# sp-uhh/audio-visual-vad

Hardware: AMD Instinct MI355X
Metric: AV frame-pairs/sec (fwd+bwd) (higher is better)
Workload: dtype f32; 1 GPU; AV_net fused training step (WaveNet-W0 encoder + ResNet-18 trunk + concat + 2xLSTM1024 + FC, masked BCE, backward, RCCL all-reduce, fused Adam): BASELINE configs[3]/[4] per-GPU shard; per_gpu_frame_pairs=1024, global_frame_pairs=1024, sequences_per_gpu=64, parallelism=dp1, reserved_cus=0, reported_block=median

## Files before the change

audio-visual-vad_amd/csrc/common.h:

```cpp
#pragma once
#include <hip/hip_runtime.h>
#include <stdint.h>
#include <atomic>

#include "avvad.h"

typedef float f32x16 __attribute__((ext_vector_type(16)));
typedef float f32x4 __attribute__((ext_vector_type(4)));

#include <stdio.h>
#define AVVAD_LAUNCH_CHECK()                                                                      \
  do {                                                                                            \
    hipError_t e_ = hipGetLastError();                                                            \
    if (e_ != hipSuccess) {                                                                       \
      fprintf(stderr, "avvad: HIP error '%s' after launch at %s:%d\n", hipGetErrorString(e_), __FILE__, __LINE__); \
      return AVVAD_ELAUNCH;                                                                       \
    }                                                                                             \
  } while (0)

#define AVVAD_ENTER() (void)hipGetLastError()

struct AvvadTune {
  int igemm_variant;
  int no_streamk;
  int kmajor;
  int lstm_no_fused_step;
  int lstm_no_persistent;
  int no_stem_kernel;
  int no_tall;
  int wn_no_fused_tail;
  int wn_no_tail_pair;
  int wn_no_fused_wgrad;
  int no_fixup1;
  int no_buf;
  int wn_flat;
  int wn_dx;
  int wn_grid;
  int wn_bwd_t;
  int bf16;
  int stagger;
  int cls_cap;
  int no_cls;
  int no_fused_stats;
  int no_s2_cls;
  int no_conv64;
  int bwd_max_cus;
  int max_cus;
};
AvvadTune& avvad_tune();
struct BwdCuCap {
  int saved;
  BwdCuCap() : saved(avvad_tune().max_cus) {
    const int b = avvad_tune().bwd_max_cus;
    if (b > 0 && (saved <= 0 || b < saved)) avvad_tune().max_cus = b;
  }
  ~BwdCuCap() { avvad_tune().max_cus = saved; }
};
static inline int grid_cus() {
  const int m = avvad_tune().max_cus;
  return (m > 0 && m < 256) ? m : 256;
}

template <auto Kernel>
int allow_large_lds(size_t bytes, size_t limit) {
  if (bytes <= 64 * 1024) return AVVAD_OK;
// ... 78 lines not shown
```

audio-visual-vad_amd/csrc/misc.hip:

```cpp
#include "common.h"

extern "C" const char* avvad_version(void) { return "avvad-hip 0.1 (gfx950, fp32 MFMA)"; }
extern "C" int avvad_abi_version(void) { return AVVAD_ABI_VERSION; }

#include <stdlib.h>
#include <string.h>
namespace {
struct OptName { const char* name; const char* env; int AvvadTune::*field; };
const OptName kOpts[] = {
    {"igemm_variant", "AVVAD_IGEMM_VARIANT", &AvvadTune::igemm_variant},
    {"no_streamk", "AVVAD_NO_STREAMK", &AvvadTune::no_streamk},
    {"kmajor", "AVVAD_KMAJOR", &AvvadTune::kmajor},
    {"lstm_no_fused_step", "AVVAD_LSTM_NO_FUSED_STEP", &AvvadTune::lstm_no_fused_step},
    {"lstm_no_persistent", "AVVAD_LSTM_NO_PERSISTENT", &AvvadTune::lstm_no_persistent},
    {"no_stem_kernel", "AVVAD_NO_STEM_KERNEL", &AvvadTune::no_stem_kernel},
    {"no_tall", "AVVAD_NO_TALL", &AvvadTune::no_tall},
    {"wn_no_fused_tail", "AVVAD_WN_NO_FUSED_TAIL", &AvvadTune::wn_no_fused_tail},
    {"wn_no_tail_pair", "AVVAD_WN_NO_TAIL_PAIR", &AvvadTune::wn_no_tail_pair},
    {"wn_no_fused_wgrad", "AVVAD_WN_NO_FUSED_WGRAD", &AvvadTune::wn_no_fused_wgrad},
    {"wn_bwd_t", "AVVAD_WN_BWD_T", &AvvadTune::wn_bwd_t},
    {"no_buf", "AVVAD_NO_BUF", &AvvadTune::no_buf},
    {"no_fixup1", "AVVAD_NO_FIXUP1", &AvvadTune::no_fixup1},
    {"no_conv64", "AVVAD_NO_CONV64", &AvvadTune::no_conv64},
    {"no_s2_cls", "AVVAD_NO_S2_CLS", &AvvadTune::no_s2_cls},
    {"wn_flat", "AVVAD_WN_FLAT", &AvvadTune::wn_flat},
    {"wn_grid", "AVVAD_WN_GRID", &AvvadTune::wn_grid},
    {"wn_dx", "AVVAD_WN_DX", &AvvadTune::wn_dx},
    {"bf16", "AVVAD_BF16", &AvvadTune::bf16},
    {"no_fused_stats", "AVVAD_NO_FUSED_STATS", &AvvadTune::no_fused_stats},
    {"no_cls", "AVVAD_NO_CLS", &AvvadTune::no_cls},
    {"cls_cap", "AVVAD_CLS_CAP", &AvvadTune::cls_cap},
    {"stagger", "AVVAD_STAGGER", &AvvadTune::stagger},
    {"max_cus", "AVVAD_MAX_CUS", &AvvadTune::max_cus},
    {"bwd_max_cus", "AVVAD_BWD_MAX_CUS", &AvvadTune::bwd_max_cus},
};
int parse_opt(const char* name, const char* v) {
  if (!strcmp(name, "igemm_variant")) return v[0] == 'd' ? 0 : (v[0] == 's' ? 1 : (v[0] == 'w' ? 2 : atoi(v)));
  if (!strcmp(name, "no_streamk")) return v[0] == 'a' ? 1 : (v[0] >= '0' && v[0] <= '9' && !v[1] ? 10 + (v[0] - '0') : atoi(v));
  if (!strcmp(name, "max_cus") || !strcmp(name, "bwd_max_cus") || !strcmp(name, "wn_flat") || !strcmp(name, "wn_grid") || !strcmp(name, "wn_dx") || !strcmp(name, "wn_bwd_t") || !strcmp(name, "no_fixup1") || !strcmp(name, "cls_cap")) return atoi(v);
  return (v[0] && strcmp(v, "0")) ? 1 : 0;
}
}

AvvadTune& avvad_tune() {
  static AvvadTune t = [] {
    AvvadTune x;
    memset(&x, 0, sizeof(x));
    x.igemm_variant = -1;
    for (const OptName& o : kOpts) {
      const char* v = getenv(o.env);
      if (v && v[0]) x.*(o.field) = parse_opt(o.name, v);
    }
// ... 281 lines not shown
```

audio-visual-vad_amd/csrc/wavenet.hip:

```cpp
#include "gemm_api.h"
#include "wn_block.h"
#include "wn_tail.h"

namespace {

static inline int grid1(long n) { long b = (n + 255) / 256; return (int)(b > 8192 ? 8192 : (b < 1 ? 1 : b)); }

__global__ void conv1d_fwd_generic(const float* __restrict__ x, const float* __restrict__ w, const float* __restrict__ bias,
                                   const float* __restrict__ res, float* __restrict__ y, int B, int Cin, int Cout, int Lin,
                                   int Lout, int fw, int dil, int relu_in, int res_off, int res_L) {
  const long n = (long)B * Cout * Lout;
  for (long i = (long)blockIdx.x * blockDim.x + threadIdx.x; i < n; i += (long)gridDim.x * blockDim.x) {
    const int t = (int)(i % Lout);
    const int co = (int)((i / Lout) % Cout);
    const int b = (int)(i / ((long)Lout * Cout));
    float acc = bias ? bias[co] : 0.f;
    const float* xb = x + (long)b * Cin * Lin + t;
    const float* wr = w + (long)co * Cin * fw;
    for (int ci = 0; ci < Cin; ++ci)
      for (int k = 0; k < fw; ++k) {
        float v = xb[(long)ci * Lin + k * dil];
        if (relu_in) v = fmaxf(v, 0.f);
        acc = fmaf(wr[ci * fw + k], v, acc);
      }
// ... 449 lines not shown
    const float* sp = s_in + (long)b * 32 * Lin + (ok ? t : 0);
    const float* rp = dS_out + (long)b * 32 * Lo + (okr ? t - dil : 0);
#pragma unroll
    for (int r = 0; r < 16; ++r) { svn[r] = sp[(long)mfma32_row(r, lh) * Lin]; rvn[r] = rp[(long)mfma32_row(r, lh) * Lo]; }
  };
  const TileWalk tw = xcd_walk(ntiles);
  if (tw.first < tw.last) issue(tw.first);
  for (long tile = tw.first; tile < tw.last; tile += tw.stride) {
    const TilePos p = tile_pos(tile, tiles_per_seq, li, Lin);
    const int b = p.b, t = p.t;
    const bool ok = p.ok;
    const int to = t - lh * dil;
    const bool okz = ok && to >= 0 && to < Lo;
    const bool okr = ok && t >= dil;
    float dz[32], sv[16], rv[16];
#pragma unroll
    for (int s = 0; s < 32; ++s) dz[s] = okz ? dzn[s] : 0.f;
#pragma unroll
    for (int r = 0; r < 16; ++r) { sv[r] = svn[r]; rv[r] = okr ? rvn[r] : 0.f; }
    issue(tile + tw.stride);
    f32x16 acc;
#pragma unroll
    for (int r = 0; r < 16; ++r) acc[r] = 0.f;
#pragma unroll
    for (int s = 0; s < 32; ++s) acc = mfma32(wt[s], dz[s], acc);
    float* op = dS_in + (long)b * 32 * Lin + t;
#pragma unroll
    for (int r = 0; r < 16; ++r)
      if (ok) op[(long)mfma32_row(r, lh) * Lin] = (sv[r] > 0.f ? acc[r] : 0.f) + rv[r];
  }
}

struct DxTile { float dz[32], sv[16], rv[16]; };
template <bool RESIDENT>
__device__ __forceinline__ void wn_block_bwd_dx_body(float* wl, const float* __restrict__ DZ, const float* __restrict__ s_in,
                                                     const float* __restrict__ dS_out, const float* __restrict__ w_dil,
                                                     float* __restrict__ dS_in, int B, int Lin, int dil) {
  const int lane = threadIdx.x & 63;
  const int li = lane & 31, lh = lane >> 5;
  const int Lo = Lin - dil;
  const int tiles_per_seq = tiles_per_sequence<32>(Lin);
  const int ntiles = B * tiles_per_seq;
  const float* wtl = wl + li * 2 + lh;
  const int rowL = Lin * 4, rowO = Lo * 4;
  float wt[32];
  auto issue = [&](int tile, DxTile& n) __attribute__((always_inline)) {
    const TilePos p = tile_pos(RESIDENT && tile >= ntiles ? ntiles - 1 : tile, tiles_per_seq, li, Lin);
    const int t = p.t;
    const int to = t - lh * dil;
    const bool okz = p.ok && to >= 0 && to < Lo;
    const bool okr = p.ok && t >= dil;
    const __amdgpu_buffer_rsrc_t rz = brsrc(DZ + (long)p.b * 32 * Lo, 32 * rowO);
    const __amdgpu_buffer_rsrc_t rs = brsrc(s_in + (long)p.b * 32 * Lin, 32 * rowL);
    const __amdgpu_buffer_rsrc_t rg = brsrc(dS_out + (long)p.b * 32 * Lo, 32 * rowO);
    const int offz = okz ? to * 4 : BUF_OOB;
    const int offs = p.ok ? t * 4 + 4 * lh * rowL : BUF_OOB;
    const int offg = okr ? (t - dil) * 4 + 4 * lh * rowO : BUF_OOB;
#pragma unroll
    for (int s = 0; s < 32; ++s) n.dz[s] = bload(rz, offz, s * rowO);
#pragma unroll
    for (int r = 0; r < 16; ++r) { n.sv[r] = bload(rs, offs, mfma32_row(r, 0) * rowL); n.rv[r] = bload(rg, offg, mfma32_row(r, 0) * rowO); }
  };
  auto compute = [&](int tile, const DxTile& c) __attribute__((always_inline)) {
    const TilePos p = tile_pos(tile, tiles_per_seq, li, Lin);
    const __amdgpu_buffer_rsrc_t ro = brsrc(dS_in + (long)p.b * 32 * Lin, 32 * rowL);
    const int offs = p.ok ? p.t * 4 + 4 * lh * rowL : BUF_OOB;
    f32x16 acc;
#pragma unroll
    for (int r = 0; r < 16; ++r) acc[r] = 0.f;
#pragma unroll
    for (int s = 0; s < 32; ++s) acc = mfma32(RESIDENT ? wt[s] : wtl[WIMG_DIL_PITCH * s], c.dz[s], acc);
#pragma unroll
    for (int r = 0; r < 16; ++r) bstore((c.sv[r] > 0.f ? acc[r] : 0.f) + c.rv[r], ro, offs, mfma32_row(r, 0) * rowL);
  };
  const TileWalkI w = xcd_walk_i(ntiles);
  DxTile ta, tb;
  if (RESIDENT && w.first < w.last) issue(w.first, ta);
  stage_w_dil(wl, w_dil, threadIdx.x, 256);
  __syncthreads();
  if (RESIDENT) {
#pragma unroll
    for (int s = 0; s < 32; ++s) wt[s] = wtl[WIMG_DIL_PITCH * s];
    pingpong_tiles<false>(w, ta, tb, issue, compute);
  } else {
    plain_tiles<false, DxTile>(w, issue, compute);
  }
}

__global__ void __launch_bounds__(256)
    wn_block_bwd_dx_buf(const float* __restrict__ DZ, const float* __restrict__ s_in, const float* __restrict__ dS_out,
                        const float* __restrict__ w_dil, float* __restrict__ dS_in, int B, int Lin, int dil) {
  __shared__ float wl[WIMG_DIL_SIZE];
  wn_block_bwd_dx_body<true>(wl, DZ, s_in, dS_out, w_dil, dS_in, B, Lin, dil);
}

__global__ void __launch_bounds__(256, 4)
    wn_block_bwd_dx_occ(const float* __restrict__ DZ, const float* __restrict__ s_in, const float* __restrict__ dS_out,
                        const float* __restrict__ w_dil, float* __restrict__ dS_in, int B, int Lin, int dil) {
  __shared__ float wl[WIMG_DIL_SIZE];
  wn_block_bwd_dx_body<false>(wl, DZ, s_in, dS_out, w_dil, dS_in, B, Lin, dil);
}

constexpr int WG_SLAB = 3 * 1024 + 64;
constexpr int WG_MAXBLK = 512;

__global__ void __launch_bounds__(256)
    wn_block_wgrad_mfma(const float* __restrict__ dS, const float* __restrict__ Z, const float* __restrict__ DZ,
                        const float* __restrict__ s_in, float* __restrict__ slab, int B, int Lin, int dil) {
// ... 47 lines not shown
    xpose(v0, ok, false, fa);
#pragma unroll
    for (int q = 0; q < 16; ++q) bs_dz += fa[q];
    xpose(v1, ok, true, fb);
#pragma unroll
    for (int q = 0; q < 16; ++q) acc0 = mfma32(fa[q], fb[q], acc0);
    xpose(v2, ok, true, fb);
#pragma unroll
    for (int q = 0; q < 16; ++q) acc1 = mfma32(fa[q], fb[q], acc1);
    xpose(v3, ok, false, fa);
#pragma unroll
    for (int q = 0; q < 16; ++q) bs_ds += fa[q];
    xpose(v4, ok, true, fb);
#pragma unroll
    for (int q = 0; q < 16; ++q) acc2 = mfma32(fa[q], fb[q], acc2);
  }

  __syncthreads();
#pragma unroll
  for (int r = 0; r < 16; ++r) {
    const int row = mfma32_row(r, lh);
    atomicAdd(&red[row * 32 + li], acc0[r]);
    atomicAdd(&red[1024 + row * 32 + li], acc1[r]);
    atomicAdd(&red[2048 + row * 32 + li], acc2[r]);
  }
  atomicAdd(&red[3072 + li], bs_dz);
  atomicAdd(&red[3104 + li], bs_ds);
  __syncthreads();
  float* out = slab + (long)blockIdx.x * WG_SLAB;
  for (int i = threadIdx.x; i < WG_SLAB; i += 256) out[i] = red[i];
}

struct DzwTile { float g[16], x[32]; };
template <bool RESIDENT>
__device__ __forceinline__ void wn_block_bwd_dz_wgrad_body(float* tiles, float* red, float* wl, float* wtl,
                                                           const float* __restrict__ dS, const float* __restrict__ w_dil,
                                                           const float* __restrict__ b_dil, const float* __restrict__ w_dense,
                                                           const float* __restrict__ s_in, float* __restrict__ DZ,
                                                           float* __restrict__ slab, int B, int Lin, int dil) {
  const int lane = threadIdx.x & 63, wave = threadIdx.x >> 6;
  const int li = lane & 31, lh = lane >> 5;
  const int Lo = Lin - dil;
  const int tiles_per_seq = tiles_per_sequence<32>(Lo);
  const int ntiles = B * tiles_per_seq;
  float* T = tiles + wave * 2 * 1056;
  float* T1 = T + 1056;
  float* Th = T + lh * 1056;
  stage_w_dil(wl, w_dil, threadIdx.x, 256);
  stage_bias(wl + WIMG_DIL_SIZE, b_dil, threadIdx.x);
  if (RESIDENT) stage_w_dense(T, w_dense, lane, 64);
  else stage_w_dense(wtl, w_dense, threadIdx.x, 256);
  for (int i = threadIdx.x; i < WG_SLAB; i += 256) red[i] = 0.f;
  __syncthreads();
  const float* wtp = (RESIDENT ? T : wtl) + lh * WIMG_DENSE_PITCH + li;
  const float* wdp = wl + li * WIMG_DIL_PITCH + lh;
  const float* bzl = wl + WIMG_DIL_SIZE + 4 * lh;
  float wt[16], wd[32];
  if (RESIDENT) {
#pragma unroll
    for (int s = 0; s < 16; ++s) wt[s] = wtp[2 * WIMG_DENSE_PITCH * s];
#pragma unroll
    for (int s = 0; s < 32; ++s) wd[s] = wdp[2 * s];
  }
  __builtin_amdgcn_wave_barrier();

  f32x16 acc0, acc1, acc2;
#pragma unroll
  for (int r = 0; r < 16; ++r) { acc0[r] = 0.f; acc1[r] = 0.f; acc2[r] = 0.f; }
  float bs_dz = 0.f, bs_ds = 0.f;
  const int rowL = Lin * 4, rowO = Lo * 4;

  auto issue = [&](int tile, DzwTile& n) __attribute__((always_inline)) {
    const TilePos p = tile_pos(tile < ntiles ? tile : ntiles - 1, tiles_per_seq, li, Lo);
    const __amdgpu_buffer_rsrc_t rg = brsrc(dS + (long)p.b * 32 * Lo, 32 * rowO);
    const __amdgpu_buffer_rsrc_t rx = brsrc(s_in + (long)p.b * 32 * Lin, 32 * rowL);
    const int offg = p.ok ? p.t * 4 + lh * rowO : BUF_OOB;
    const int offx = p.ok ? (p.t + lh * dil) * 4 : BUF_OOB;
#pragma unroll
    for (int q = 0; q < 16; ++q) n.g[q] = bload(rg, offg, 2 * q * rowO);
#pragma unroll
    for (int c = 0; c < 32; ++c) n.x[c] = bload(rx, offx, c * rowL);
  };
  auto compute = [&](int tidx, const DzwTile& c) __attribute__((always_inline)) {
    const TilePos p = tile_pos(tidx, tiles_per_seq, li, Lo);
    const int offo = p.ok ? p.t * 4 + 4 * lh * rowO : BUF_OOB;
    const __amdgpu_buffer_rsrc_t rz = brsrc(DZ + (long)p.b * 32 * Lo, 32 * rowO);
    float x[32];
#pragma unroll
    for (int s = 0; s < 32; ++s) x[s] = relu1(c.x[s]);
    f32x16 z;
#pragma unroll
    for (int r = 0; r < 16; ++r) z[r] = bzl[mfma32_row(r, 0)];
#pragma unroll
    for (int s = 0; s < 32; ++s) z = mfma32(RESIDENT ? wd[s] : wdp[2 * s], x[s], z);
    f32x16 acc;
#pragma unroll
    for (int r = 0; r < 16; ++r) acc[r] = 0.f;
#pragma unroll
    for (int q = 0; q < 16; ++q) acc = mfma32(RESIDENT ? wt[q] : wtp[2 * WIMG_DENSE_PITCH * q], c.g[q], acc);
    float f0[16], f1[16];
    __builtin_amdgcn_wave_barrier();
#pragma unroll
    for (int r = 0; r < 16; ++r) {
      const float dz = z[r] > 0.f ? acc[r] : 0.f;
      bstore(dz, rz, offo, mfma32_row(r, 0) * rowO);
      T[mfma32_row(r, lh) * 33 + li] = dz;
    }
    __builtin_amdgcn_wave_barrier();
#pragma unroll
    for (int q = 0; q < 16; ++q) { f0[q] = T[li * 33 + 2 * q + lh]; bs_dz += f0[q]; }
    __builtin_amdgcn_wave_barrier();
#pragma unroll
    for (int s = 0; s < 32; ++s) Th[s * 33 + li] = x[s];
    __builtin_amdgcn_wave_barrier();
#pragma unroll
    for (int q = 0; q < 16; ++q) f1[q] = T[li * 33 + 2 * q + lh];
#pragma unroll
    for (int q = 0; q < 16; ++q) acc0 = mfma32(f0[q], f1[q], acc0);
#pragma unroll
    for (int q = 0; q < 16; ++q) f1[q] = T1[li * 33 + 2 * q + lh];
#pragma unroll
    for (int q = 0; q < 16; ++q) acc1 = mfma32(f0[q], f1[q], acc1);
    __builtin_amdgcn_wave_barrier();
#pragma unroll
    for (int q = 0; q < 16; ++q) T[(2 * q + lh) * 33 + li] = c.g[q];
#pragma unroll
    for (int r = 0; r < 16; ++r) T1[mfma32_row(r, lh) * 33 + li] = relu1(z[r]);
    __builtin_amdgcn_wave_barrier();
#pragma unroll
    for (int q = 0; q < 16; ++q) { f0[q] = T[li * 33 + 2 * q + lh]; bs_ds += f0[q]; }
#pragma unroll
    for (int q = 0; q < 16; ++q) f1[q] = T1[li * 33 + 2 * q + lh];
#pragma unroll
    for (int q = 0; q < 16; ++q) acc2 = mfma32(f0[q], f1[q], acc2);
    __builtin_amdgcn_wave_barrier();
  };
  const TileWalkI w = xcd_walk_i(ntiles);
  DzwTile ta, tb;
  if (RESIDENT) {
    if (w.first < w.last) issue(w.first, ta);
    pingpong_tiles<true>(w, ta, tb, issue, compute);
  } else {
    plain_tiles<true, DzwTile>(w, issue, compute);
  }

  for (int wv = 0; wv < 4; ++wv) {
    __syncthreads();
    if (wave == wv) {
#pragma unroll
      for (int r = 0; r < 16; ++r) {
        const int row = mfma32_row(r, lh);
        red[row * 32 + li] += acc0[r];
        red[1024 + row * 32 + li] += acc1[r];
        red[2048 + row * 32 + li] += acc2[r];
      }
      if (lh == 0) { red[3072 + li] += bs_dz; red[3104 + li] += bs_ds; }
      __builtin_amdgcn_wave_barrier();
      if (lh == 1) { red[3072 + li] += bs_dz; red[3104 + li] += bs_ds; }
    }
  }
  __syncthreads();
  float* out = slab + (long)blockIdx.x * WG_SLAB;
  for (int i = threadIdx.x; i < WG_SLAB; i += 256) out[i] = red[i];
}

__global__ void __launch_bounds__(256)
    wn_block_bwd_dz_wgrad_mfma(const float* __restrict__ dS, const float* __restrict__ w_dil, const float* __restrict__ b_dil,
                               const float* __restrict__ w_dense, const float* __restrict__ s_in, float* __restrict__ DZ,
                               float* __restrict__ slab, int B, int Lin, int dil) {
  __shared__ float tile[4 * 2 * 32 * 33];
  __shared__ float red[WG_SLAB];
  __shared__ float wl[WIMG_DIL_SIZE + 32];
  wn_block_bwd_dz_wgrad_body<true>(tile, red, wl, nullptr, dS, w_dil, b_dil, w_dense, s_in, DZ, slab, B, Lin, dil);
}

__global__ void __launch_bounds__(256, 2)
    wn_block_bwd_dz_wgrad_occ(const float* __restrict__ dS, const float* __restrict__ w_dil, const float* __restrict__ b_dil,
                               const float* __restrict__ w_dense, const float* __restrict__ s_in, float* __restrict__ DZ,
                               float* __restrict__ slab, int B, int Lin, int dil) {
  __shared__ float tile[4 * 2 * 32 * 33];
  __shared__ float red[WG_SLAB];
  __shared__ float wl[WIMG_DIL_SIZE + 32];
  __shared__ float wtl[WIMG_DENSE_SIZE];
  wn_block_bwd_dz_wgrad_body<false>(tile, red, wl, wtl, dS, w_dil, b_dil, w_dense, s_in, DZ, slab, B, Lin, dil);
}

typedef float f4u __attribute__((ext_vector_type(4), aligned(4)));

__global__ void __launch_bounds__(256, 2)
    wn_block_bwd_dzw_t(const float* __restrict__ dS, const float* __restrict__ w_dil, const float* __restrict__ b_dil,
                       const float* __restrict__ w_dense, const float* __restrict__ s_in, float* __restrict__ DZ,
                       float* __restrict__ slab, int B, int Lin, int dil) {
  __shared__ float red[WG_SLAB];
  __shared__ float wl[WIMG_BDENSE];
  const int lane = threadIdx.x & 63;
  const int li = lane & 31, lh = lane >> 5;
  const int Lo = Lin - dil;
  const int tiles_per_seq = tiles_per_sequence<32>(Lo);
  const long ntiles = (long)B * tiles_per_seq;
  const long wave0 = ((long)blockIdx.x * blockDim.x + threadIdx.x) >> 6;
  const long nwaves = ((long)gridDim.x * blockDim.x) >> 6;
  stage_w_dil(wl + WIMG_DIL, w_dil, threadIdx.x, 256);
  stage_w_dense(wl + WIMG_DENSE, w_dense, threadIdx.x, 256);
  stage_bias(wl + WIMG_BDIL, b_dil, threadIdx.x);
  for (int i = threadIdx.x; i < WG_SLAB; i += 256) red[i] = 0.f;
  __syncthreads();
  const float* wdp = wl + WIMG_DIL + li * WIMG_DIL_PITCH + lh;
  const float* wtp = wl + WIMG_DENSE + lh * WIMG_DENSE_PITCH + li;
  const float bz = wl[WIMG_BDIL + li];

  f32x16 acc0, acc1, acc2;
#pragma unroll
  for (int r = 0; r < 16; ++r) { acc0[r] = 0.f; acc1[r] = 0.f; acc2[r] = 0.f; }
  float bs_dz = 0.f, bs_ds = 0.f;

  for (long tl = wave0; tl < ntiles; tl += nwaves) {
    const TilePos p = tile_pos(tl, tiles_per_seq, li, Lo);
// ... 190 lines not shown
    return {FwdForm::WIDE, wn_grid_size((long)B * cdiv(Lo, 128), 4, t.wn_grid > 0 ? t.wn_grid : 1024, 0, XcdRound::UP)};
  const long ntiles = (long)B * cdiv(Lo, 32);
  if (buf && t.wn_flat == 5 && Lo >= 32)
    return {FwdForm::DMA, wn_grid_size(ntiles, 8, 512, t.wn_grid, XcdRound::UP_FROM_8)};
  if (buf && (t.wn_flat == 0 || t.wn_flat == 4))
    return {FwdForm::OCC, wn_grid_size(ntiles, 4, 1024, t.wn_grid, XcdRound::UP_FROM_8)};
  return {buf ? FwdForm::BUF : FwdForm::FLAT, wn_grid_size(ntiles, 4, 512, t.wn_grid, XcdRound::NONE)};
}

static DxChoice dx_form(int B, int Lin) {
  const AvvadTune& t = avvad_tune();
  const long ntiles = (long)B * cdiv(Lin, 32);
  if (buf_ok(B, Lin) && (t.wn_dx == 0 || t.wn_dx == 2))
    return {DxForm::OCC, wn_grid_size(ntiles, 4, 1024, 0, XcdRound::UP_FROM_8)};
  return {buf_ok(B, Lin) && t.wn_dx != 3 ? DxForm::BUF : DxForm::FLAT, wn_grid_size(ntiles, 4, 512, 0, XcdRound::NONE)};
}

static BwdChoice bwd_form(int B, int Lo, bool shared_device, bool any_grad) {
  const AvvadTune& t = avvad_tune();
  const long ntiles = (long)B * cdiv(Lo, 32);
  if (!any_grad || t.wn_no_fused_wgrad)
    return {BwdForm::UNFUSED, wn_grid_size(ntiles, 16, WG_MAXBLK, 0, XcdRound::NONE), wn_grid_size(ntiles, 4, 512, 0, XcdRound::NONE),
            wn_grid_size(ntiles, 4, 768, 0, XcdRound::NONE)};
  switch (t.wn_bwd_t == 0 ? (shared_device ? 3 : 2) : t.wn_bwd_t) {
    case 3:
      return {BwdForm::RESIDENT, wn_grid_size(ntiles, 16, 256, 0, XcdRound::NONE), 0, 0};
    case 2:
      return {BwdForm::OCC, wn_grid_size(ntiles, 16, WG_MAXBLK, 0, XcdRound::DOWN_FROM_8), 0, 0};
    default:
      return {BwdForm::TRANSPOSED, wn_grid_size(ntiles, 16, WG_MAXBLK, 0, XcdRound::NONE), 0, 0};
  }
}

static TailFwdChoice tail_fwd_form(int B, int R, int Bn, int P) {
  if (!(R == 32 && Bn % 32 == 0)) return {TailFwdForm::GENERIC, 0};
  const int nt = Bn % 128 == 0 ? 4 : 1;
  return {nt == 4 ? TailFwdForm::MFMA4 : TailFwdForm::MFMA1, wn_grid_size((long)B * P * (Bn / (32 * nt)), 4, 2048, 0, XcdRound::NONE)};
}

static TailBwdChoice tail_bwd_form(int B, int Lv, int R, int Bn, int P, bool any_grad) {
  const AvvadTune& t = avvad_tune();
  const long ntiles = (long)B * cdiv(Lv, 32);
  if (!(R == 32 && Bn % 32 == 0 && Bn <= 1024) || P > Lv) return {TailBwdForm::GENERIC, 0};
  if (Bn == 256 && any_grad && !t.wn_no_fused_tail)
    return {t.wn_no_tail_pair ? TailBwdForm::FUSED : TailBwdForm::PAIR, wn_grid_size(ntiles, 4, TAIL_MAXBLK, 0, XcdRound::NONE)};
  return {TailBwdForm::MFMA, wn_grid_size(ntiles, 4, 2048, 0, XcdRound::NONE)};
}

static void launch_block_fwd(const float* s_in, const float* wd, const float* bd, const float* we, const float* be, float* s_out,
                             int B, int Lin, int dil, hipStream_t s) {
  const FwdChoice c = fwd_form(B, Lin, dil);
  const dim3 grid(c.grid);
  switch (c.form) {
    case FwdForm::WIDE: hipLaunchKernelGGL(wn_block_fwd_w4, grid, dim3(256), 0, s, s_in, wd, bd, we, be, s_out, B, Lin, dil); break;
    case FwdForm::DMA: hipLaunchKernelGGL(wn_block_fwd_dma, grid, dim3(512), 0, s, s_in, wd, bd, we, be, s_out, B, Lin, dil); break;
    case FwdForm::OCC: hipLaunchKernelGGL(wn_block_fwd_occ, grid, dim3(256), 0, s, s_in, wd, bd, we, be, s_out, B, Lin, dil); break;
    case FwdForm::BUF: hipLaunchKernelGGL(wn_block_fwd_buf, grid, dim3(256), 0, s, s_in, wd, bd, we, be, s_out, B, Lin, dil); break;
    case FwdForm::FLAT:
      hipLaunchKernelGGL(wn_block_fwd_mfma<0>, grid, dim3(256), 0, s, s_in, wd, bd, we, be, s_out, (float*)nullptr, B, Lin, dil);
      break;
  }
}

static int wgrad_conv1d(const float* dy, const float* x, float* dw, int B, int Cout, int Cin, int Lout, int Lin, int fw,
                        int dil, int relu_in, hipStream_t s, float* slab) {
  const long K = (long)B * Lout;
// ... 81 lines not shown
                         prm->dil_w_h[i], bd, (const float*)nullptr, z, B, R, D, p.L[i], p.L[i + 1], fw, dil, 1, 0, 0);
      hipLaunchKernelGGL(conv1d_fwd_generic, dim3(grid1((long)B * R * p.L[i + 1])), dim3(256), 0, s, z, prm->dense_w_h[i], be,
                         ws + p.s[i], ws + p.s[i + 1], B, D, R, p.L[i + 1], p.L[i + 1], 1, 1, 1, p.L[i] - p.L[i + 1], p.L[i]);
    }
  }
  launch_tail_fwd(ws + p.s[p.n], prm->bott_w, d->use_bias ? prm->bott_b : (const float*)nullptr, out, B, R, d->Bn, p.L[p.n],
                  d->P, s);
  AVVAD_LAUNCH_CHECK();
  return AVVAD_OK;
}

extern "C" int avvad_wavenet_block_fwd(const float* s_in, const float* w_dil, const float* b_dil, const float* w_dense,
                                       const float* b_dense, float* s_out, int B, int Lin, int dil, avvad_stream_t sv) {
  AVVAD_ENTER();
  if (!s_in || !w_dil || !w_dense || !s_out || B <= 0 || dil < 1 || Lin - dil < 1) return AVVAD_EINVAL;
  launch_block_fwd(s_in, w_dil, b_dil, w_dense, b_dense, s_out, B, Lin, dil, (hipStream_t)sv);
  AVVAD_LAUNCH_CHECK();
  return AVVAD_OK;
}

extern "C" int avvad_wavenet_bwd(const float* wave, const avvad_wavenet_params* prm, const float* dout,
                                 const avvad_wavenet_grads* g, float* dwave, const avvad_wavenet_desc* d, void* wsv,
                                 size_t ws_bytes, avvad_stream_t sv) {
  AVVAD_ENTER();
  Plan p;
  if (!wave || !prm || !dout || !g || !wsv || ws_misaligned(wsv) || make_plan(d, &p) || !d->save_for_backward) return AVVAD_EINVAL;
  if (ws_bytes < p.total * sizeof(float)) return AVVAD_EWORKSPACE;
  hipStream_t s = (hipStream_t)sv;
  float* ws = (float*)wsv;
  const int B = d->B, R = d->R, D = d->D, fw = d->fw, Bn = d->Bn;
  int rc;
  float* Z = ws + p.z;
  float* DZ = ws + p.dz;
  float* GA = ws + p.ga;
  float* GB = ws + p.gb;
  if ((rc = launch_tail_bwd(ws + p.s[p.n], prm->bott_w, d->use_bias ? prm->bott_b : (const float*)nullptr, dout, g->bott_w,
                            d->use_bias ? g->bott_b : (float*)nullptr, GA, ws + p.dzt, ws + p.slab, ws + p.gslab, B, R, Bn,
                            p.L[p.n], d->P, s)))
    return rc;
  WgradTab wtab;
  bool any_slab = false;
  for (int l = 0; l < WN_MAXL; ++l) {
    wtab.slab[l] = nullptr; wtab.nslab[l] = 0;
    wtab.dW_dil[l] = wtab.db_dil[l] = wtab.dW_dense[l] = wtab.db_dense[l] = nullptr;
  }
  auto note_slabs = [&](int i, float* slab_i, int wb) {
    wtab.slab[i] = slab_i; wtab.nslab[i] = wb;
    wtab.dW_dil[i] = g->dil_w_h[i]; wtab.dW_dense[i] = g->dense_w_h[i];
    wtab.db_dil[i] = d->use_bias ? g->dil_b_h[i] : (float*)nullptr;
    wtab.db_dense[i] = d->use_bias ? g->dense_b_h[i] : (float*)nullptr;
    any_slab = true;
  };
  for (int i = p.n - 1; i >= 0; --i) {
    float* const slab_i = ws + p.slab + (size_t)i * WG_MAXBLK * WG_SLAB;
    const int dil = d->dilations_h[i];
    const int Li = p.L[i], Lo = p.L[i + 1];
    const float* si = ws + p.s[i];
    const float* bd = d->use_bias ? prm->dil_b_h[i] : nullptr;
    const bool fast = mfma_shape(d);
    float* Zi = fast ? ws + p.zs[i] : Z;
    if (!fast)
      hipLaunchKernelGGL(conv1d_fwd_generic, dim3(grid1((long)B * D * Lo)), dim3(256), 0, s, si, prm->dil_w_h[i], bd,
                         (const float*)nullptr, Zi, B, R, D, Li, Lo, fw, dil, 1, 0, 0);
    if (fast) {
      const bool any_grad = g->dil_w_h[i] || g->dense_w_h[i] || (d->use_bias && (g->dil_b_h[i] || g->dense_b_h[i]));
      const BwdChoice bc = bwd_form(B, Lo, d->shared_device != 0, any_grad);
      switch (bc.form) {
        case BwdForm::RESIDENT:
          hipLaunchKernelGGL(wn_block_bwd_dz_wgrad_mfma, dim3(bc.grid), dim3(256), 0, s, GA, prm->dil_w_h[i], bd,
                             prm->dense_w_h[i], si, DZ, slab_i, B, Li, dil);
          break;
        case BwdForm::OCC:
          hipLaunchKernelGGL(wn_block_bwd_dz_wgrad_occ, dim3(bc.grid), dim3(256), 0, s, GA, prm->dil_w_h[i], bd,
                             prm->dense_w_h[i], si, DZ, slab_i, B, Li, dil);
          break;
        case BwdForm::TRANSPOSED:
          hipLaunchKernelGGL(wn_block_bwd_dzw_t, dim3(bc.grid), dim3(256), 0, s, GA, prm->dil_w_h[i], bd, prm->dense_w_h[i], si,
                             DZ, slab_i, B, Li, dil);
          break;
        case BwdForm::UNFUSED:
          hipLaunchKernelGGL(wn_block_fwd_mfma<2>, dim3(bc.grid_z), dim3(256), 0, s, si, prm->dil_w_h[i], bd, prm->dense_w_h[i],
                             (const float*)nullptr, (float*)nullptr, Zi, B, Li, dil);
          hipLaunchKernelGGL(wn_block_bwd_dz_mfma, dim3(bc.grid_dz), dim3(256), 0, s, GA, Zi, prm->dense_w_h[i], DZ, B, Lo);
          if (any_grad)
            hipLaunchKernelGGL(wn_block_wgrad_mfma, dim3(bc.grid), dim3(256), 0, s, GA, Zi, DZ, si, slab_i, B, Li, dil);
          break;
      }
      if (any_grad) note_slabs(i, slab_i, bc.grid);
      const DxChoice dc = dx_form(B, Li);
      switch (dc.form) {
        case DxForm::OCC:
          hipLaunchKernelGGL(wn_block_bwd_dx_occ, dim3(dc.grid), dim3(256), 0, s, DZ, si, GA, prm->dil_w_h[i], GB, B, Li, dil);
          break;
        case DxForm::BUF:
          hipLaunchKernelGGL(wn_block_bwd_dx_buf, dim3(dc.grid), dim3(256), 0, s, DZ, si, GA, prm->dil_w_h[i], GB, B, Li, dil);
          break;
        case DxForm::FLAT:
          hipLaunchKernelGGL(wn_block_bwd_dx_mfma, dim3(dc.grid), dim3(256), 0, s, DZ, si, GA, prm->dil_w_h[i], GB, B, Li, dil);
          break;
      }
    } else {
      if (g->dense_w_h[i] && (rc = wgrad_conv1d(GA, Zi, g->dense_w_h[i], B, R, D, Lo, Lo, 1, 1, 1, s, ws + p.gslab))) return rc;
      if (d->use_bias) bias_grad(GA, g->dense_b_h[i], B, R, Lo, s);
      hipLaunchKernelGGL(conv1d_bwd_data_generic, dim3(grid1((long)B * D * Lo)), dim3(256), 0, s, GA, prm->dense_w_h[i], Zi,
                         (const float*)nullptr, DZ, B, D, R, Lo, Lo, 1, 1, 0, 0);
      if (g->dil_w_h[i] && (rc = wgrad_conv1d(DZ, si, g->dil_w_h[i], B, D, R, Lo, Li, fw, dil, 1, s, ws + p.gslab))) return rc;
      if (d->use_bias) bias_grad(DZ, g->dil_b_h[i], B, D, Lo, s);
      hipLaunchKernelGGL(conv1d_bwd_data_generic, dim3(grid1((long)B * R * Li)), dim3(256), 0, s, DZ, prm->dil_w_h[i], si, GA,
                         GB, B, R, D, Li, Lo, fw, dil, Li - Lo, Lo);
    }
    float* t = GA; GA = GB; GB = t;
  }
  if (any_slab) hipLaunchKernelGGL(wn_wgrad_reduce_all, dim3(WG_SLAB / 32, p.n), dim3(256), 0, s, wtab);
  if (d->qc * fw <= 4) {
    if (g->causal_w || (d->use_bias && g->causal_b))
    {
      const int ny = B < 32 ? B : 32;
      float* part = ws + p.gslab;
      hipLaunchKernelGGL(narrow_conv1d_grads, dim3(R, ny), dim3(256), 0, s, GA, wave, part, B, R, d->qc, p.L[0], d->L, fw);
      hipLaunchKernelGGL(narrow_conv1d_grads_sum, dim3(cdiv(R * 5, 256)), dim3(256), 0, s, part, ny, R, d->qc * fw, g->causal_w,
                         d->use_bias ? g->causal_b : (float*)nullptr);
    }
  } else {
// ... 10 lines not shown
```

audio-visual-vad_amd/csrc/wn_block.h:

```cpp
#pragma once
#include "common.h"

constexpr int WIMG_DIL_PITCH = 65, WIMG_DENSE_PITCH = 33;
constexpr int WIMG_DIL = 0;
constexpr int WIMG_DENSE = WIMG_DIL + 32 * WIMG_DIL_PITCH;
constexpr int WIMG_BDIL = WIMG_DENSE + 32 * WIMG_DENSE_PITCH;
constexpr int WIMG_BDENSE = WIMG_BDIL + 32;
constexpr int WIMG_SIZE = WIMG_BDENSE + 32;
constexpr int WIMG_DIL_SIZE = WIMG_DENSE;
constexpr int WIMG_DENSE_SIZE = 32 * WIMG_DENSE_PITCH;

__device__ __forceinline__ void stage_w_dil(float* img, const float* __restrict__ w_dil, int tid, int nthreads) {
  for (int i = tid; i < 2048; i += nthreads) img[(i >> 6) * WIMG_DIL_PITCH + (i & 63)] = w_dil[i];
}
__device__ __forceinline__ void stage_w_dense(float* img, const float* __restrict__ w_dense, int tid, int nthreads) {
  for (int i = tid; i < 1024; i += nthreads) img[(i >> 5) * WIMG_DENSE_PITCH + (i & 31)] = w_dense[i];
}
__device__ __forceinline__ void stage_bias(float* img, const float* __restrict__ b, int tid) {
  if (tid < 32) img[tid] = b ? b[tid] : 0.f;
}
__device__ __forceinline__ void stage_block_weights(float* img, const float* __restrict__ w_dil, const float* __restrict__ b_dil,
                                                    const float* __restrict__ w_dense, const float* __restrict__ b_dense,
                                                    int tid, int nthreads) {
  stage_w_dil(img + WIMG_DIL, w_dil, tid, nthreads);
  stage_w_dense(img + WIMG_DENSE, w_dense, tid, nthreads);
  stage_bias(img + WIMG_BDIL, b_dil, tid);
  stage_bias(img + WIMG_BDENSE, b_dense, tid);
}

template <int W>
__device__ __forceinline__ int tiles_per_sequence(int L) { return (L + W - 1) >> __builtin_ctz(W); }
struct TilePos { int b, t0, t; bool ok; };
template <int W = 32, class I>
__device__ __forceinline__ TilePos tile_pos(I tile, int tiles_per_seq, int lane_off, int L) {
  TilePos p;
  p.b = (int)(tile / tiles_per_seq);
  p.t0 = (int)(tile - (I)p.b * tiles_per_seq) * W;
  p.t = p.t0 + lane_off;
  p.ok = p.t < L;
  return p;
}

template <bool PIN, class Set, class Issue, class Compute>
__device__ __forceinline__ void pingpong_tiles(const TileWalkI& w, Set& a, Set& b, Issue issue, Compute compute) {
  for (int tile = w.first; tile < w.last; tile += 2 * w.stride) {
    issue(tile + w.stride, b);
    if (PIN) __builtin_amdgcn_sched_barrier(0);
    compute(tile, a);
    if (tile + w.stride >= w.last) break;
    issue(tile + 2 * w.stride, a);
    if (PIN) __builtin_amdgcn_sched_barrier(0);
    compute(tile + w.stride, b);
  }
}
template <bool PIN, class Set, class Issue, class Compute>
__device__ __forceinline__ void plain_tiles(const TileWalkI& w, Issue issue, Compute compute) {
  for (int tile = w.first; tile < w.last; tile += w.stride) {
    Set a;
    issue(tile, a);
    if (PIN) __builtin_amdgcn_sched_barrier(0);
    compute(tile, a);
  }
}
```

Before: 60070 frame-pairs/s.

## Fuse WaveNet block dx backward with next block's dz/wgrad in one paired kernel

```diff
diff --git a/audio-visual-vad_amd/csrc/common.h b/audio-visual-vad_amd/csrc/common.h
--- a/audio-visual-vad_amd/csrc/common.h
+++ b/audio-visual-vad_amd/csrc/common.h
@@ -30,7 +30,7 @@
   int no_tall;
   int wn_no_fused_tail;
   int wn_no_tail_pair;
-  int wn_no_fused_wgrad;
+  int wn_no_fused_wgrad, wn_no_pair;
   int no_fixup1;
   int no_buf;
   int wn_flat;
diff --git a/audio-visual-vad_amd/csrc/misc.hip b/audio-visual-vad_amd/csrc/misc.hip
--- a/audio-visual-vad_amd/csrc/misc.hip
+++ b/audio-visual-vad_amd/csrc/misc.hip
@@ -18,6 +18,7 @@
     {"wn_no_fused_tail", "AVVAD_WN_NO_FUSED_TAIL", &AvvadTune::wn_no_fused_tail},
     {"wn_no_tail_pair", "AVVAD_WN_NO_TAIL_PAIR", &AvvadTune::wn_no_tail_pair},
     {"wn_no_fused_wgrad", "AVVAD_WN_NO_FUSED_WGRAD", &AvvadTune::wn_no_fused_wgrad},
+    {"wn_no_pair", "AVVAD_WN_NO_PAIR", &AvvadTune::wn_no_pair},
     {"wn_bwd_t", "AVVAD_WN_BWD_T", &AvvadTune::wn_bwd_t},
     {"no_buf", "AVVAD_NO_BUF", &AvvadTune::no_buf},
     {"no_fixup1", "AVVAD_NO_FIXUP1", &AvvadTune::no_fixup1},
diff --git a/audio-visual-vad_amd/csrc/wavenet.hip b/audio-visual-vad_amd/csrc/wavenet.hip
--- a/audio-visual-vad_amd/csrc/wavenet.hip
+++ b/audio-visual-vad_amd/csrc/wavenet.hip
@@ -505,20 +505,17 @@
 }
 
 struct DxTile { float dz[32], sv[16], rv[16]; };
-template <bool RESIDENT>
-__device__ __forceinline__ void wn_block_bwd_dx_body(float* wl, const float* __restrict__ DZ, const float* __restrict__ s_in,
-                                                     const float* __restrict__ dS_out, const float* __restrict__ w_dil,
-                                                     float* __restrict__ dS_in, int B, int Lin, int dil) {
-  const int lane = threadIdx.x & 63;
-  const int li = lane & 31, lh = lane >> 5;
-  const int Lo = Lin - dil;
-  const int tiles_per_seq = tiles_per_sequence<32>(Lin);
-  const int ntiles = B * tiles_per_seq;
-  const float* wtl = wl + li * 2 + lh;
-  const int rowL = Lin * 4, rowO = Lo * 4;
-  float wt[32];
-  auto issue = [&](int tile, DxTile& n) __attribute__((always_inline)) {
-    const TilePos p = tile_pos(RESIDENT && tile >= ntiles ? ntiles - 1 : tile, tiles_per_seq, li, Lin);
+struct DxPieces {
+  const float* DZ; const float* s_in; const float* dS_out; float* dS_in;
+  int Lin, Lo, dil, li, lh, tiles_per_seq, ntiles, rowL, rowO;
+  __device__ __forceinline__ DxPieces(const float* DZ_, const float* s_in_, const float* dS_out_, float* dS_in_, int B, int Lin_,
+                                      int dil_)
+      : DZ(DZ_), s_in(s_in_), dS_out(dS_out_), dS_in(dS_in_), Lin(Lin_), Lo(Lin_ - dil_), dil(dil_), li(threadIdx.x & 31),
+        lh((threadIdx.x & 63) >> 5), tiles_per_seq(tiles_per_sequence<32>(Lin_)), ntiles(B * tiles_per_sequence<32>(Lin_)),
+        rowL(Lin_ * 4), rowO((Lin_ - dil_) * 4) {}
+  template <bool CLAMP>
+  __device__ __forceinline__ void issue(int tile, DxTile& n) const {
+    const TilePos p = tile_pos(CLAMP && tile >= ntiles ? ntiles - 1 : tile, tiles_per_seq, li, Lin);
     const int t = p.t;
     const int to = t - lh * dil;
     const bool okz = p.ok && to >= 0 && to < Lo;
@@ -533,8 +530,9 @@
     for (int s = 0; s < 32; ++s) n.dz[s] = bload(rz, offz, s * rowO);
 #pragma unroll
     for (int r = 0; r < 16; ++r) { n.sv[r] = bload(rs, offs, mfma32_row(r, 0) * rowL); n.rv[r] = bload(rg, offg, mfma32_row(r, 0) * rowO); }
-  };
-  auto compute = [&](int tile, const DxTile& c) __attribute__((always_inline)) {
+  }
+  template <class WFrag>
+  __device__ __forceinline__ void compute(int tile, const DxTile& c, WFrag wfrag, float (&out)[16]) const {
     const TilePos p = tile_pos(tile, tiles_per_seq, li, Lin);
     const __amdgpu_buffer_rsrc_t ro = brsrc(dS_in + (long)p.b * 32 * Lin, 32 * rowL);
     const int offs = p.ok ? p.t * 4 + 4 * lh * rowL : BUF_OOB;
@@ -542,11 +540,27 @@
 #pragma unroll
     for (int r = 0; r < 16; ++r) acc[r] = 0.f;
 #pragma unroll
-    for (int s = 0; s < 32; ++s) acc = mfma32(RESIDENT ? wt[s] : wtl[WIMG_DIL_PITCH * s], c.dz[s], acc);
-#pragma unroll
-    for (int r = 0; r < 16; ++r) bstore((c.sv[r] > 0.f ? acc[r] : 0.f) + c.rv[r], ro, offs, mfma32_row(r, 0) * rowL);
+    for (int s = 0; s < 32; ++s) acc = mfma32(wfrag(s), c.dz[s], acc);
+#pragma unroll
+    for (int r = 0; r < 16; ++r) {
+      out[r] = (c.sv[r] > 0.f ? acc[r] : 0.f) + c.rv[r];
+      bstore(out[r], ro, offs, mfma32_row(r, 0) * rowL);
+    }
+  }
+};
+template <bool RESIDENT>
+__device__ __forceinline__ void wn_block_bwd_dx_body(float* wl, const float* __restrict__ DZ, const float* __restrict__ s_in,
+                                                     const float* __restrict__ dS_out, const float* __restrict__ w_dil,
+                                                     float* __restrict__ dS_in, int B, int Lin, int dil) {
+  const DxPieces dx(DZ, s_in, dS_out, dS_in, B, Lin, dil);
+  const float* wtl = wl + dx.li * 2 + dx.lh;
+  float wt[32];
+  auto issue = [&](int tile, DxTile& n) __attribute__((always_inline)) { dx.issue<RESIDENT>(tile, n); };
+  auto compute = [&](int tile, const DxTile& c) __attribute__((always_inline)) {
+    float out[16];
+    dx.compute(tile, c, [&](int s) __attribute__((always_inline)) { return RESIDENT ? wt[s] : wtl[WIMG_DIL_PITCH * s]; }, out);
   };
-  const TileWalkI w = xcd_walk_i(ntiles);
+  const TileWalkI w = xcd_walk_i(dx.ntiles);
   DxTile ta, tb;
   if (RESIDENT && w.first < w.last) issue(w.first, ta);
   stage_w_dil(wl, w_dil, threadIdx.x, 256);
@@ -660,17 +674,28 @@
 }
 
 struct DzwTile { float g[16], x[32]; };
-template <bool RESIDENT>
+struct PairTile { DxTile up; float x[32]; };
+struct PairUp {
+  const float* DZ; const float* s_in; const float* dS_out; const float* w_dil; float* dS_in; int dil;
+};
+template <bool RESIDENT, bool PAIRED = false>
 __device__ __forceinline__ void wn_block_bwd_dz_wgrad_body(float* tiles, float* red, float* wl, float* wtl,
                                                            const float* __restrict__ dS, const float* __restrict__ w_dil,
                                                            const float* __restrict__ b_dil, const float* __restrict__ w_dense,
                                                            const float* __restrict__ s_in, float* __restrict__ DZ,
-                                                           float* __restrict__ slab, int B, int Lin, int dil) {
+                                                           float* __restrict__ slab, int B, int Lin, int dil,
+                                                           const PairUp pu = PairUp{}) {
+  static_assert(!(RESIDENT && PAIRED), "the paired kernel holds no weights in registers");
+  using Tile = typename std::conditional<PAIRED, PairTile, DzwTile>::type;
   const int lane = threadIdx.x & 63, wave = threadIdx.x >> 6;
   const int li = lane & 31, lh = lane >> 5;
   const int Lo = Lin - dil;
   const int tiles_per_seq = tiles_per_sequence<32>(Lo);
   const int ntiles = B * tiles_per_seq;
+  const DxPieces up(pu.DZ, pu.s_in, pu.dS_out, pu.dS_in, B, Lo, pu.dil);
+  float* const wlu = red;
+  const float* wul = wlu + li * 2 + lh;
+  if (PAIRED) stage_w_dil(wlu, pu.w_dil, threadIdx.x, 256);
   float* T = tiles + wave * 2 * 1056;
   float* T1 = T + 1056;
   float* Th = T + lh * 1056;
@@ -678,7 +703,8 @@
   stage_bias(wl + WIMG_DIL_SIZE, b_dil, threadIdx.x);
   if (RESIDENT) stage_w_dense(T, w_dense, lane, 64);
   else stage_w_dense(wtl, w_dense, threadIdx.x, 256);
-  for (int i = threadIdx.x; i < WG_SLAB; i += 256) red[i] = 0.f;
+  if (!PAIRED)
+    for (int i = threadIdx.x; i < WG_SLAB; i += 256) red[i] = 0.f;
   __syncthreads();
   const float* wtp = (RESIDENT ? T : wtl) + lh * WIMG_DENSE_PITCH + li;
   const float* wdp = wl + li * WIMG_DIL_PITCH + lh;
@@ -698,21 +724,34 @@
   float bs_dz = 0.f, bs_ds = 0.f;
   const int rowL = Lin * 4, rowO = Lo * 4;
 
-  auto issue = [&](int tile, DzwTile& n) __attribute__((always_inline)) {
+  auto issue = [&](int tile, Tile& n) __attribute__((always_inline)) {
     const TilePos p = tile_pos(tile < ntiles ? tile : ntiles - 1, tiles_per_seq, li, Lo);
-    const __amdgpu_buffer_rsrc_t rg = brsrc(dS + (long)p.b * 32 * Lo, 32 * rowO);
     const __amdgpu_buffer_rsrc_t rx = brsrc(s_in + (long)p.b * 32 * Lin, 32 * rowL);
-    const int offg = p.ok ? p.t * 4 + lh * rowO : BUF_OOB;
     const int offx = p.ok ? (p.t + lh * dil) * 4 : BUF_OOB;
-#pragma unroll
-    for (int q = 0; q < 16; ++q) n.g[q] = bload(rg, offg, 2 * q * rowO);
+    if constexpr (PAIRED) {
+      up.issue<false>(tile, n.up);
+    } else {
+      const __amdgpu_buffer_rsrc_t rg = brsrc(dS + (long)p.b * 32 * Lo, 32 * rowO);
+      const int offg = p.ok ? p.t * 4 + lh * rowO : BUF_OOB;
+#pragma unroll
+      for (int q = 0; q < 16; ++q) n.g[q] = bload(rg, offg, 2 * q * rowO);
+    }
 #pragma unroll
     for (int c = 0; c < 32; ++c) n.x[c] = bload(rx, offx, c * rowL);
   };
-  auto compute = [&](int tidx, const DzwTile& c) __attribute__((always_inline)) {
+  auto compute = [&](int tidx, const Tile& c) __attribute__((always_inline)) {
     const TilePos p = tile_pos(tidx, tiles_per_seq, li, Lo);
     const int offo = p.ok ? p.t * 4 + 4 * lh * rowO : BUF_OOB;
     const __amdgpu_buffer_rsrc_t rz = brsrc(DZ + (long)p.b * 32 * Lo, 32 * rowO);
+    float g[16];
+    if constexpr (PAIRED) {
+      float d[16];
+      up.compute(tidx, c.up, [&](int s) __attribute__((always_inline)) { return wul[WIMG_DIL_PITCH * s]; }, d);
+      d_rows_to_k_pairs(d, g);
+    } else {
+#pragma unroll
+      for (int q = 0; q < 16; ++q) g[q] = c.g[q];
+    }
     float x[32];
 #pragma unroll
     for (int s = 0; s < 32; ++s) x[s] = relu1(c.x[s]);
@@ -725,7 +764,7 @@
 #pragma unroll
     for (int r = 0; r < 16; ++r) acc[r] = 0.f;
 #pragma unroll
-    for (int q = 0; q < 16; ++q) acc = mfma32(RESIDENT ? wt[q] : wtp[2 * WIMG_DENSE_PITCH * q], c.g[q], acc);
+    for (int q = 0; q < 16; ++q) acc = mfma32(RESIDENT ? wt[q] : wtp[2 * WIMG_DENSE_PITCH * q], g[q], acc);
     float f0[16], f1[16];
     __builtin_amdgcn_wave_barrier();
 #pragma unroll
@@ -751,7 +790,7 @@
     for (int q = 0; q < 16; ++q) acc1 = mfma32(f0[q], f1[q], acc1);
     __builtin_amdgcn_wave_barrier();
 #pragma unroll
-    for (int q = 0; q < 16; ++q) T[(2 * q + lh) * 33 + li] = c.g[q];
+    for (int q = 0; q < 16; ++q) T[(2 * q + lh) * 33 + li] = g[q];
 #pragma unroll
     for (int r = 0; r < 16; ++r) T1[mfma32_row(r, lh) * 33 + li] = relu1(z[r]);
     __builtin_amdgcn_wave_barrier();
@@ -764,12 +803,16 @@
     __builtin_amdgcn_wave_barrier();
   };
   const TileWalkI w = xcd_walk_i(ntiles);
-  DzwTile ta, tb;
+  Tile ta, tb;
   if (RESIDENT) {
     if (w.first < w.last) issue(w.first, ta);
     pingpong_tiles<true>(w, ta, tb, issue, compute);
   } else {
-    plain_tiles<true, DzwTile>(w, issue, compute);
+    plain_tiles<true, Tile>(w, issue, compute);
+  }
+  if (PAIRED) {
+    __syncthreads();
+    for (int i = threadIdx.x; i < WG_SLAB; i += 256) red[i] = 0.f;
   }
 
   for (int wv = 0; wv < 4; ++wv) {
@@ -811,6 +854,20 @@
   __shared__ float wl[WIMG_DIL_SIZE + 32];
   __shared__ float wtl[WIMG_DENSE_SIZE];
   wn_block_bwd_dz_wgrad_body<false>(tile, red, wl, wtl, dS, w_dil, b_dil, w_dense, s_in, DZ, slab, B, Lin, dil);
+}
+
+__global__ void __launch_bounds__(256, 2)
+    wn_block_bwd_pair(const float* __restrict__ dz_up, const float* __restrict__ s_up, const float* __restrict__ dS_res,
+                      const float* __restrict__ w_dil_up, float* __restrict__ dS_up, int dil_up,
+                      const float* __restrict__ w_dil, const float* __restrict__ b_dil, const float* __restrict__ w_dense,
+                      const float* __restrict__ s_in, float* __restrict__ DZ, float* __restrict__ slab, int B, int Lin, int dil) {
+  __shared__ float tile[4 * 2 * 32 * 33];
+  __shared__ float red[WG_SLAB];
+  __shared__ float wl[WIMG_DIL_SIZE + 32];
+  __shared__ float wtl[WIMG_DENSE_SIZE];
+  static_assert(WIMG_DIL_SIZE <= WG_SLAB, "the upper block's weight image lives in red[]");
+  wn_block_bwd_dz_wgrad_body<false, true>(tile, red, wl, wtl, nullptr, w_dil, b_dil, w_dense, s_in, DZ, slab, B, Lin, dil,
+                                          PairUp{dz_up, s_up, dS_res, w_dil_up, dS_up, dil_up});
 }
 
 typedef float f4u __attribute__((ext_vector_type(4), aligned(4)));
@@ -1067,6 +1124,14 @@
   }
 }
 
+struct PairChoice { bool pair; int grid; };
+static PairChoice pair_form(int B, int Lprev, int Lp, bool shared_device, bool any_grad) {
+  if (avvad_tune().wn_no_pair || shared_device || Lp < 32 || !buf_ok(B, Lprev)) return {false, 0};
+  const BwdForm bw = bwd_form(B, Lp, shared_device, any_grad).form;
+  if (dx_form(B, Lp).form == DxForm::FLAT || (bw != BwdForm::RESIDENT && bw != BwdForm::OCC)) return {false, 0};
+  return {true, wn_grid_size((long)B * cdiv(Lp, 32), 16, WG_MAXBLK, 0, XcdRound::DOWN_FROM_8)};
+}
+
 static TailFwdChoice tail_fwd_form(int B, int R, int Bn, int P) {
   if (!(R == 32 && Bn % 32 == 0)) return {TailFwdForm::GENERIC, 0};
   const int nt = Bn % 128 == 0 ? 4 : 1;
@@ -1214,6 +1279,7 @@
   int rc;
   float* Z = ws + p.z;
   float* DZ = ws + p.dz;
+  float* DZn = Z;
   float* GA = ws + p.ga;
   float* GB = ws + p.gb;
   if ((rc = launch_tail_bwd(ws + p.s[p.n], prm->bott_w, d->use_bias ? prm->bott_b : (const float*)nullptr, dout, g->bott_w,
@@ -1233,6 +1299,10 @@
     wtab.db_dense[i] = d->use_bias ? g->dense_b_h[i] : (float*)nullptr;
     any_slab = true;
   };
+  auto wants_grad = [&](int i) {
+    return g->dil_w_h[i] || g->dense_w_h[i] || (d->use_bias && (g->dil_b_h[i] || g->dense_b_h[i]));
+  };
+  bool dz_ready = false;
   for (int i = p.n - 1; i >= 0; --i) {
     float* const slab_i = ws + p.slab + (size_t)i * WG_MAXBLK * WG_SLAB;
     const int dil = d->dilations_h[i];
@@ -1245,32 +1315,44 @@
       hipLaunchKernelGGL(conv1d_fwd_generic, dim3(grid1((long)B * D * Lo)), dim3(256), 0, s, si, prm->dil_w_h[i], bd,
                          (const float*)nullptr, Zi, B, R, D, Li, Lo, fw, dil, 1, 0, 0);
     if (fast) {
-      const bool any_grad = g->dil_w_h[i] || g->dense_w_h[i] || (d->use_bias && (g->dil_b_h[i] || g->dense_b_h[i]));
-      const BwdChoice bc = bwd_form(B, Lo, d->shared_device != 0, any_grad);
-      switch (bc.form) {
-        case BwdForm::RESIDENT:
-          hipLaunchKernelGGL(wn_block_bwd_dz_wgrad_mfma, dim3(bc.grid), dim3(256), 0, s, GA, prm->dil_w_h[i], bd,
-                             prm->dense_w_h[i], si, DZ, slab_i, B, Li, dil);
-          break;
-        case BwdForm::OCC:
-          hipLaunchKernelGGL(wn_block_bwd_dz_wgrad_occ, dim3(bc.grid), dim3(256), 0, s, GA, prm->dil_w_h[i], bd,
-                             prm->dense_w_h[i], si, DZ, slab_i, B, Li, dil);
-          break;
-        case BwdForm::TRANSPOSED:
-          hipLaunchKernelGGL(wn_block_bwd_dzw_t, dim3(bc.grid), dim3(256), 0, s, GA, prm->dil_w_h[i], bd, prm->dense_w_h[i], si,
-                             DZ, slab_i, B, Li, dil);
-          break;
-        case BwdForm::UNFUSED:
-          hipLaunchKernelGGL(wn_block_fwd_mfma<2>, dim3(bc.grid_z), dim3(256), 0, s, si, prm->dil_w_h[i], bd, prm->dense_w_h[i],
-                             (const float*)nullptr, (float*)nullptr, Zi, B, Li, dil);
-          hipLaunchKernelGGL(wn_block_bwd_dz_mfma, dim3(bc.grid_dz), dim3(256), 0, s, GA, Zi, prm->dense_w_h[i], DZ, B, Lo);
-          if (any_grad)
-            hipLaunchKernelGGL(wn_block_wgrad_mfma, dim3(bc.grid), dim3(256), 0, s, GA, Zi, DZ, si, slab_i, B, Li, dil);
-          break;
+      if (!dz_ready) {
+        const bool any_grad = wants_grad(i);
+        const BwdChoice bc = bwd_form(B, Lo, d->shared_device != 0, any_grad);
+        switch (bc.form) {
+          case BwdForm::RESIDENT:
+            hipLaunchKernelGGL(wn_block_bwd_dz_wgrad_mfma, dim3(bc.grid), dim3(256), 0, s, GA, prm->dil_w_h[i], bd,
+                               prm->dense_w_h[i], si, DZ, slab_i, B, Li, dil);
+            break;
+          case BwdForm::OCC:
+            hipLaunchKernelGGL(wn_block_bwd_dz_wgrad_occ, dim3(bc.grid), dim3(256), 0, s, GA, prm->dil_w_h[i], bd,
+                               prm->dense_w_h[i], si, DZ, slab_i, B, Li, dil);
+            break;
+          case BwdForm::TRANSPOSED:
+            hipLaunchKernelGGL(wn_block_bwd_dzw_t, dim3(bc.grid), dim3(256), 0, s, GA, prm->dil_w_h[i], bd, prm->dense_w_h[i], si,
+                               DZ, slab_i, B, Li, dil);
+            break;
+          case BwdForm::UNFUSED:
+            hipLaunchKernelGGL(wn_block_fwd_mfma<2>, dim3(bc.grid_z), dim3(256), 0, s, si, prm->dil_w_h[i], bd, prm->dense_w_h[i],
+                               (const float*)nullptr, (float*)nullptr, Zi, B, Li, dil);
+            hipLaunchKernelGGL(wn_block_bwd_dz_mfma, dim3(bc.grid_dz), dim3(256), 0, s, GA, Zi, prm->dense_w_h[i], DZ, B, Lo);
+            if (any_grad)
+              hipLaunchKernelGGL(wn_block_wgrad_mfma, dim3(bc.grid), dim3(256), 0, s, GA, Zi, DZ, si, slab_i, B, Li, dil);
+            break;
+        }
+        if (any_grad) note_slabs(i, slab_i, bc.grid);
       }
-      if (any_grad) note_slabs(i, slab_i, bc.grid);
+      const PairChoice pc = i > 0 ? pair_form(B, p.L[i - 1], Li, d->shared_device != 0, wants_grad(i - 1)) : PairChoice{false, 0};
+      dz_ready = pc.pair;
+      if (pc.pair) {
+        float* const slab_p = ws + p.slab + (size_t)(i - 1) * WG_MAXBLK * WG_SLAB;
+        hipLaunchKernelGGL(wn_block_bwd_pair, dim3(pc.grid), dim3(256), 0, s, DZ, si, GA, prm->dil_w_h[i], GB, dil,
+                           prm->dil_w_h[i - 1], d->use_bias ? prm->dil_b_h[i - 1] : (const float*)nullptr, prm->dense_w_h[i - 1],
+                           ws + p.s[i - 1], DZn, slab_p, B, p.L[i - 1], d->dilations_h[i - 1]);
+        note_slabs(i - 1, slab_p, pc.grid);
+        float* t = DZ; DZ = DZn; DZn = t;
+      }
       const DxChoice dc = dx_form(B, Li);
-      switch (dc.form) {
+      if (!pc.pair) switch (dc.form) {
         case DxForm::OCC:
           hipLaunchKernelGGL(wn_block_bwd_dx_occ, dim3(dc.grid), dim3(256), 0, s, DZ, si, GA, prm->dil_w_h[i], GB, B, Li, dil);
           break;
diff --git a/audio-visual-vad_amd/csrc/wn_block.h b/audio-visual-vad_amd/csrc/wn_block.h
--- a/audio-visual-vad_amd/csrc/wn_block.h
+++ b/audio-visual-vad_amd/csrc/wn_block.h
@@ -41,6 +41,17 @@
   return p;
 }
 
+__device__ __forceinline__ void d_rows_to_k_pairs(const float (&d)[16], float (&g)[16]) {
+#pragma unroll
+  for (int r = 0; r < 16; r += 2) {
+    const int q = mfma32_row(r, 0) >> 1;
+    const auto sw = __builtin_amdgcn_permlane32_swap(__builtin_bit_cast(unsigned, d[r]), __builtin_bit_cast(unsigned, d[r + 1]),
+                                                     false, false);
+    g[q] = __builtin_bit_cast(float, (unsigned)sw[0]);
+    g[q + 2] = __builtin_bit_cast(float, (unsigned)sw[1]);
+  }
+}
+
 template <bool PIN, class Set, class Issue, class Compute>
 __device__ __forceinline__ void pingpong_tiles(const TileWalkI& w, Set& a, Set& b, Issue issue, Compute compute) {
   for (int tile = w.first; tile < w.last; tile += 2 * w.stride) {
```

Result: no change. 60040 frame-pairs/s (median of 2 runs) (-0.0%).
